# michaelnny/alpha_zero

Measured on AMD Instinct MI355X. Metric: self-play moves/sec (whole node), 9x9 Go @ 200 sims/move, higher is better.
Workload: dtype fp32-class evaluator (f16 hi+lo pairs, 3 MFMA products, fp32 accumulate) / f32-f64 tree

## Files before the change

alpha_zero_amd/csrc/azsp_hip.hip:

```cpp
#include <hip/hip_runtime.h>
#include <stdlib.h>

#include <type_traits>

#include "azsp_impl.h"
#include "az_conv64.h"
#include "az_conv19.h"
#include "az_conv_sp.h"
#include "az_conv_sp17.h"
#include "az_resblock_sp17.h"
#include "az_conv_sp2.h"
#include "az_conv_spg.h"
#include "az_stem_spg.h"

static hipError_t g_last = hipSuccess;
#define AZ_HIP(x) ((g_last = (x)) == hipSuccess ? 0 : -1)

template <int N, int GAME, class Op>
__global__ void __launch_bounds__(256) k_game(const AzCfg c, const AzMem m, const Op op, const int g0, const int g1) {
    __shared__ typename Engine<WaveDev, N, GAME>::SC sc[4];
    const int wave = (int)(threadIdx.x >> 6);
    const int g = g0 + (int)blockIdx.x * 4 + wave;
    if (g >= g1) return;
    Engine<WaveDev, N, GAME> e(c, m, g, sc[wave]);
    op(e);
}

__global__ void __launch_bounds__(256) k_dihedral(const DihedralArgs a, long long total) {
    for (long long t = (long long)blockIdx.x * blockDim.x + threadIdx.x; t < total; t += (long long)gridDim.x * blockDim.x)
        az_dihedral_elem(a, t);
}

__global__ void __launch_bounds__(256) k_replay_gather(const ReplayGatherArgs a, long long total) {
    for (long long t = (long long)blockIdx.x * blockDim.x + threadIdx.x; t < total; t += (long long)gridDim.x * blockDim.x)
        az_replay_gather_elem(a, t);
}

__global__ void __launch_bounds__(256) k_bias_act(const BiasActArgs a) {
    for (long long i = (long long)blockIdx.x * blockDim.x + threadIdx.x; i < a.nvec; i += (long long)gridDim.x * blockDim.x)
        az_bias_act_vec(a, i);
}

__global__ void __launch_bounds__(1024) k_harvest_scan(const int* __restrict__ len, int* __restrict__ ofs, int* __restrict__ counts, int n2, int rot,
                                                        int cap, int max_games) {
    __shared__ int ss[1024], sg[1024], best[2];
    const int t = (int)threadIdx.x, per = (n2 + 1023) / 1024, lo = t * per < n2 ? t * per : n2, hi = lo + per < n2 ? lo + per : n2;
    int s = 0, g = 0;
    for (int i = lo; i < hi; ++i) {
        const int l = len[(i + rot) % n2];
        s += l;
        g += l > 0;
    }
    ss[t] = s;
    sg[t] = g;
    if (t < 2) best[t] = 0;
    __syncthreads();
    for (int d = 1; d < 1024; d <<= 1) {
        const int a = t >= d ? ss[t - d] : 0, b = t >= d ? sg[t - d] : 0;
        __syncthreads();
        ss[t] += a;
        sg[t] += b;
        __syncthreads();
    }
    int mine[2] = {0, 0};
    az_harvest_scan_range(len, ofs, n2, rot, cap, max_games, lo, hi, ss[t] - s, sg[t] - g, mine);
    if (mine[1] > 0) {
        atomicMax(&best[0], mine[0]);
        atomicMax(&best[1], mine[1]);
    }
    __syncthreads();
    if (t < 2) counts[t] = best[t];
}

namespace azb {
void* alloc(size_t n) {
    void* p = nullptr;
    if (AZ_HIP(hipMalloc(&p, n))) return nullptr;
    if (AZ_HIP(hipMemset(p, 0, n))) {
        hipFree(p);
        return nullptr;
    }
    return p;
}
void release(void* p) { (void)hipFree(p); }
int h2d(void* d, const void* s, size_t n, void* st) {
    if (AZ_HIP(hipMemcpyAsync(d, s, n, hipMemcpyHostToDevice, (hipStream_t)st))) return -1;
    return AZ_HIP(hipStreamSynchronize((hipStream_t)st));
}
int d2h(void* d, const void* s, size_t n, void* st) {
    if (AZ_HIP(hipMemcpyAsync(d, s, n, hipMemcpyDeviceToHost, (hipStream_t)st))) return -1;
    return AZ_HIP(hipStreamSynchronize((hipStream_t)st));
}
int zero(void* d, size_t n, void* st) { return AZ_HIP(hipMemsetAsync(d, 0, n, (hipStream_t)st)); }
int sync(void* st) { return AZ_HIP(hipStreamSynchronize((hipStream_t)st)); }
void* host_alloc(size_t n) {
    void* p = nullptr;
    return AZ_HIP(hipHostMalloc(&p, n, hipHostMallocDefault)) ? nullptr : p;
}
void host_release(void* p) { (void)hipHostFree(p); }
int set_device(int dev) {
    int n = 0;
    if (AZ_HIP(hipGetDeviceCount(&n)) || n < 1) return -1;
    return AZ_HIP(hipSetDevice(dev));
}
const char* backend_error() { return hipGetErrorString(g_last); }
template <class K, class... A> static int launch_k(K* kernel, unsigned grid, unsigned block, size_t lds, void* st, const A&... args) {
    hipLaunchKernelGGL(kernel, dim3(grid), dim3(block), lds, (hipStream_t)st, args...);
    return AZ_HIP(hipGetLastError());
}
template <class F> static int with_flag(bool flag, F&& f) { return flag ? f(std::true_type{}) : f(std::false_type{}); }
template <class F> static int with_flag(bool f0, bool f1, F&& f) {
    return with_flag(f0, [&](auto F0) { return with_flag(f1, [&](auto F1) { return f(decltype(F0){}, F1); }); });
}
static int cu_count() {
    static int n_cu = 0;
    if (n_cu == 0) {
        int dev = 0;
        hipDeviceProp_t prop;
        if (hipGetDevice(&dev) != hipSuccess || hipGetDeviceProperties(&prop, dev) != hipSuccess) return -1;
        n_cu = prop.multiProcessorCount > 0 ? prop.multiProcessorCount : 256;
    }
    return n_cu;
}
static int persistent_grid(long long units, int k = 1) {
    const int n_cu = cu_count();
    if (n_cu < 0) return -1;
    const long long slots = n_cu / k > 0 ? n_cu / k : 1;
    return k * (int)(units < slots ? units : slots);
}
template <int N, int GAME, class Op> int launch(const AzCfg& c, const AzMem& m, const Op& op, void* st, int g0, int g1) {
    return launch_k(k_game<N, GAME, Op>, (unsigned)((g1 - g0 + 3) / 4), 256, 0, st, c, m, op, g0, g1);
}
int launch_dihedral(const DihedralArgs& a, long long total, void* st) {
    long long blocks = (total + 255) / 256;
    if (blocks > 2048) blocks = 2048;
    return launch_k(k_dihedral, (unsigned)blocks, 256, 0, st, a, total);
}
int launch_replay_gather(const ReplayGatherArgs& a, long long total, void* st) {
    long long blocks = (total + 255) / 256;
    if (blocks > 256 * 16) blocks = 256 * 16;
    return launch_k(k_replay_gather, (unsigned)blocks, 256, 0, st, a, total);
}
int launch_harvest_scan(const int* len, int* ofs, int* counts, int n2, int rot, int cap, int max_games, void* st) {
    return launch_k(k_harvest_scan, 1, 1024, 0, st, len, ofs, counts, n2, rot, cap, max_games);
}
int launch_bias_act(const BiasActArgs& a, void* st) {
    long long blocks = (a.nvec + 255) / 256;
    if (blocks > 256 * 32) blocks = 256 * 32;
    return launch_k(k_bias_act, (unsigned)blocks, 256, 0, st, a);
}
int launch_conv3x3_tiled(const void* x, const void* w, const float* bias, const void* res, void* y, long long boards, int S, int C,
                         int relu, void* st, int f16) {
    if (f16 && (S != CV_S || C != CV_C)) return 1;
    const auto xb = (const unsigned char*)x, rb = (const unsigned char*)res;
    const auto wb = (const unsigned short*)w;
    const auto yb = (unsigned char*)y;
    if (C == C6_C && (S == 17 || S == 9)) {
        const long long ntiles = S == 17 ? boards : (boards + 2) / 3;
        const int grid = persistent_grid(ntiles);
        if (grid < 0) return -1;
        return with_flag(S == 17, res != nullptr, [&](auto G17, auto RES) {
            return launch_k(k_conv3x3_t64<C6Geo<G17 ? 17 : 9>, RES, 8>, grid, CW_THREADS, 0, st, xb, wb, bias, rb, yb, (int)ntiles, relu);
        });
    }
    if (S == C9_S && C == 256) {
        static const bool two_launch = getenv("AZSP_CONV19_TWO_LAUNCH") != nullptr;
        const int grid = persistent_grid(boards, two_launch ? 4 : 8);
        if (grid < 0) return -1;
        if (x == y || res == y) return 1;
        if (!two_launch) {
            return with_flag(res != nullptr, [&](auto RES) {
                return launch_k(k_conv3x3_op19q<RES>, grid, CW_THREADS, 0, st, xb, wb, bias, rb, yb, (int)boards, relu);
            });
        }
        const int rc = with_flag(res != nullptr, [&](auto RES) {
            return launch_k(k_conv3x3_hb19<RES, 16>, grid, CW_THREADS, 0, st, xb, wb, bias, rb, yb, (int)boards, 0, 1, 256, 0, 32, 0);
        });
        if (rc) return rc;
        return launch_k(k_conv3x3_hb19<true, 16>, grid, CW_THREADS, 0, st, xb, wb, bias, (const unsigned char*)yb, yb, (int)boards, relu, 0, 256, 128, 32, 16);
    }
    if (S != CV_S || C != CV_C) return 1;
    const long long ntiles = (boards + CV_TB - 1) / CV_TB;
    const int grid = persistent_grid(ntiles);
    if (grid < 0) return -1;
    return with_flag(res != nullptr, f16 != 0, [&](auto RES, auto F16) {
        return launch_k(k_conv3x3_tiled<RES, 16, F16>, grid, CW_THREADS, 0, st, xb, wb, bias, rb, yb, (int)ntiles, relu);
    });
}
int launch_resblock_tiled(const void* x, const void* w1, const float* b1, const void* w2, const float* b2, void* y, long long boards, int S, int C,
                          void* st) {
    if (C != C6_C || (S != 17 && S != 9)) return 1;
    const long long ntiles = S == 17 ? boards : (boards + 2) / 3;
    const int grid = persistent_grid(ntiles);
    if (grid < 0) return -1;
    return with_flag(S == 17, [&](auto G17) {
        return launch_k(k_resblock64<C6Geo<G17 ? 17 : 9>>, grid, CW_THREADS, 0, st, (const unsigned char*)x, (const unsigned short*)w1, b1,
                        (const unsigned short*)w2, b2, (unsigned char*)y, (int)ntiles);
    });
}
int launch_stem_tiled(const void* x, const void* w, const float* bias, void* y, long long boards, int S, int C, int pad, int relu, void* st, int f16) {
    if (f16 && (S != CV_S || C != CV_C || pad != 1)) return 1;
    const bool t64 = C == C6_C && ((S == 13 && pad == 3) || (S == 9 && pad == 1)), go19 = S == C9_S && C == 256 && pad == 1;
    if (!t64 && !go19 && (S != CV_S || C != CV_C || pad != 1)) return 1;
    const long long ntiles = t64 ? (S == 13 ? boards : (boards + 2) / 3) : go19 ? boards : (boards + CV_TB - 1) / CV_TB;
    const int grid = persistent_grid(ntiles, go19 ? 4 : 1);
    if (grid < 0) return -1;
    const auto xb = (const unsigned char*)x, nores = (const unsigned char*)nullptr;
    const auto wb = (const unsigned short*)w;
    const auto yb = (unsigned char*)y;
    if (t64)
        return with_flag(S == 13, [&](auto G17) {
            return launch_k(k_conv3x3_t64<C6Geo<G17 ? 17 : 9>, false, 4>, grid, CW_THREADS, 0, st, xb, wb, bias, nores, yb, (int)ntiles, relu);
        });
    if (go19) return launch_k(k_conv3x3_hb19<false, 4>, grid, CW_THREADS, 0, st, xb, wb, bias, nores, yb, (int)boards, relu, 1, 32, 0, 4, 0);
    return with_flag(f16 != 0, [&](auto F16) {
        return launch_k(k_conv3x3_tiled<false, 4, F16>, grid, CW_THREADS, 0, st, xb, wb, bias, nores, yb, (int)ntiles, relu);
    });
}
int launch_head_tiled(const void* x, const float* w, const float* bias, void* pol, void* val, long long boards, int S, int C, int npol, int nval,
                      int pol_stride, int val_stride, void* st, int f16) {
    if (C % 8 || C > 1024 || npol + nval != 3) return 1;
    const long long npos = boards * S * S;
    return with_flag(f16 != 0, [&](auto F16) {
        return launch_k(k_head_tiled<3, F16>, (unsigned)((npos + 255) / 256), 256, 0, st, (const unsigned char*)x, w, bias, (unsigned short*)pol,
                        (unsigned short*)val, npos, npol, C, S * S, cv_tile_boards(S) * S * S, pol_stride, val_stride);
    });
}
template <int T1, int T2, bool F16> static int launch_fc_heads_t(const FcHeadsArgs& a, void* st) {
    return launch_k(k_fc_heads<T1, T2, F16>, (unsigned)((a.boards + 127) / 128), 256, 0, st, (const unsigned short*)a.pol, (const unsigned short*)a.val,
                    (const unsigned short*)a.wp, a.bp, a.ks1, (const unsigned short*)a.w1, a.b1, a.ks2, a.w2, a.b2, a.priors, a.values, a.boards, a.A);
}
int launch_fc_heads(const FcHeadsArgs& a, void* st) {
    const int nt1 = (a.A + 31) / 32, nt2 = (a.F + 31) / 32;
    if (a.f16) return nt1 == 3 && nt2 == 4 ? launch_fc_heads_t<3, 4, true>(a, st) : 1;
    if (nt1 == 3 && nt2 == 2) return launch_fc_heads_t<3, 2, false>(a, st);
    if (nt1 == 3 && nt2 == 4) return launch_fc_heads_t<3, 4, false>(a, st);
    if (nt1 == 6 && nt2 == 2) return launch_fc_heads_t<6, 2, false>(a, st);
    if (nt1 == 6 && nt2 == 4) return launch_fc_heads_t<6, 4, false>(a, st);
    if (nt1 == 12 && nt2 == 8) return launch_fc_heads_t<12, 8, false>(a, st);
    return 1;
}
int launch_tile_layout(const void* src, void* dst, long long boards, int S, int C, int to_tiled, void* st) {
    if (C % 8 || S < 1) return 1;
    const int nch = C / 8, tile_rows = cv_tile_boards(S) * S * S;
    const long long nchunks = boards * S * S * nch;
    return launch_k(k_tile_layout, (unsigned)((nchunks + 255) / 256), 256, 0, st, (const unsigned char*)src, (unsigned char*)dst, nchunks, to_tiled, nch,
                    tile_rows);
}
int launch_split_layout(const void* src, void* dst, long long boards, int S, int C, int to_split, void* st, unsigned* range) {
    if (C % 8 || S < 1) return 1;
    const long long nchunks = boards * S * S * (C / 8);
    return launch_k(k_split_layout, (unsigned)((nchunks + 255) / 256), 256, 0, st, (const unsigned char*)src, (unsigned char*)dst, nchunks, to_split, C / 8,
                    S * S, range);
}
template <bool RES, int NCH, int NCG, bool XLO0 = false>
static int launch_sp(const void* x, const void* w, const float* bias, const void* res, void* y, long long boards, int relu, void* st, unsigned* range) {
    const int grid = persistent_grid(boards, NCG);
    if (grid < 0) return -1;
    return launch_k(k_conv3x3_sp<RES, NCH, NCG, XLO0>, grid, CW_THREADS, 0, st, (const unsigned char*)x, (const _Float16*)w, bias, (const unsigned char*)res,
                    (unsigned char*)y, (int)boards, relu, range);
}
template <bool RES, int NCH, bool XLO0 = false>
static int launch_sp17(const void* x, const void* w, const float* bias, const void* res, void* y, long long boards, int relu, void* st, unsigned* range) {
    const int grid = persistent_grid(boards);
    if (grid < 0) return -1;
    return launch_k(k_conv3x3_sp17<RES, NCH, XLO0>, grid, CW_THREADS, 0, st, (const unsigned char*)x, (const _Float16*)w, bias, (const unsigned char*)res,
                    (unsigned char*)y, (int)boards, relu, range);
}
template <bool RES, int KSUB, int NT, int NJ, int HALVES>
static int launch_spg_t(const void* x, const void* w, const float* bias, const void* res, void* y, long long boards, int S, int C, int relu, void* st,
                        unsigned* range) {
    const long long nct = ((long long)S * S + 15) / 16, items = boards * ((nct + NJ - 1) / NJ) * (C / (16 * NT)), grid = (items + 3) / 4;
    if (grid > 0x7fffffffLL) return 1;
    return launch_k(k_conv3x3_spg<RES, KSUB, NT, NJ, HALVES>, (unsigned)grid, 256, 0, st, (const unsigned char*)x, (const _Float16*)w, bias,
                    (const unsigned char*)(RES ? res : nullptr), (unsigned char*)y, (int)boards, S, C, relu, range);
}
template <bool RES, int KSUB, int NT, int HALVES>
static int launch_spgw_t(const void* x, const void* w, const float* bias, const void* res, void* y, long long boards, int S, int C, int relu, void* st,
                         unsigned* range) {
    const long long nct = ((long long)S * S + 15) / 16, grid = (boards * ((nct + 2) / 3) * (C / (64 * NT)) + 7) / 8 * 8;
    if (grid > 0x7fffffffLL || C % (64 * NT)) return 1;
    return launch_k(k_conv3x3_spgw<RES, KSUB, NT, HALVES>, (unsigned)grid, 256, 0, st, (const unsigned char*)x, (const _Float16*)w, bias,
                    (const unsigned char*)(RES ? res : nullptr), (unsigned char*)y, (int)boards, S, C, relu, range);
}
template <int KSUB, int HALVES>
static int launch_spg_k(const void* x, const void* w, const float* bias, const void* res, void* y, long long boards, int S, int C, int relu, void* st,
                        unsigned* range, bool latency) {
    constexpr int NT = KSUB == 2 ? 1 : 2;
    return with_flag(res != nullptr, [&](auto RES) {
        return latency ? launch_spg_t<RES, KSUB, 1, 2, HALVES>(x, w, bias, res, y, boards, S, C, relu, st, range)
                       : launch_spgw_t<RES, KSUB, NT, HALVES>(x, w, bias, res, y, boards, S, C, relu, st, range);
    });
}
static int launch_spg(const void* x, const void* w, const float* bias, const void* res, void* y, long long boards, int S, int C, int relu, void* st,
                      unsigned* range, bool latency, int halves) {
    if (S < 3 || S > 64 || boards < 1 || boards > 0x7fffffffLL) return 1;
    if (C == 64) return launch_spg_k<2, 1>(x, w, bias, res, y, boards, S, C, relu, st, range, latency);
    if (C == 128)
        return halves == 2 ? launch_spg_k<4, 2>(x, w, bias, res, y, boards, S, C, relu, st, range, latency)
                           : launch_spg_k<4, 1>(x, w, bias, res, y, boards, S, C, relu, st, range, latency);
    if (C == 256) return launch_spg_k<8, 1>(x, w, bias, res, y, boards, S, C, relu, st, range, latency);
    return 1;
}
static constexpr long long SPG_DEFAULT_WAVES = 1024;
static long long& spg_max_waves() {
    static long long n = [] {
        const char* e = getenv("AZSP_SPG_MAX_WAVES");
        const long long v = e ? atoll(e) : SPG_DEFAULT_WAVES;
        return v < 0 ? 0LL : v;
    }();
    return n;
}
static bool small_batch(long long boards, int S, int C) { return boards * ((((long long)S * S + 15) / 16 + 1) / 2) * (C / 16) <= spg_max_waves(); }
long long small_batch_waves(long long n) {
    const long long old = spg_max_waves();
    if (n >= 0) spg_max_waves() = n;
    return old;
}
int launch_conv3x3_split(const void* x, const void* w, const float* bias, const void* res, void* y, long long boards, int S, int C, int relu,
                         void* st, unsigned* range) {
    const bool sp17 = S == Sp17Geo::S && C == 64, sp9 = S == SpGeo9::S && (C == 128 || C == 64), small = small_batch(boards, S, C);
    if (!(sp17 || sp9) || small) return launch_spg(x, w, bias, res, y, boards, S, C, relu, st, range, small, sp9 && C == 128 ? 2 : 1);
    if (sp17)
        return with_flag(res != nullptr, [&](auto RES) { return launch_sp17<RES, 8>(x, w, bias, res, y, boards, relu, st, range); });
    if (C == 64) return with_flag(res != nullptr, [&](auto RES) { return launch_sp<RES, 8, 1>(x, w, bias, res, y, boards, relu, st, range); });
    const int grid = persistent_grid(boards, 2);
    if (grid < 0) return -1;
    return with_flag(res != nullptr, [&](auto RES) {
        return launch_k(k_conv3x3_sp2<RES>, grid, CW_THREADS, 0, st, (const unsigned char*)x, (const _Float16*)w, bias, (const unsigned char*)res,
                        (unsigned char*)y, (int)boards, relu, range);
    });
}
enum Scratch {
    SCRATCH_SPG_BLOCK,
    SCRATCH_SP9_TAIL,
    SCRATCH_COUNT
};
static constexpr long long SPG_SCRATCH_BOARDS = 256;
static void* device_scratch(Scratch which, size_t bytes) {
    static void* buf[SCRATCH_COUNT][16] = {};
    int dev = 0;
    if (hipGetDevice(&dev) != hipSuccess || dev < 0 || dev >= 16) return nullptr;
    if (!buf[which][dev] && AZ_HIP(hipMalloc(&buf[which][dev], bytes))) return nullptr;
    return buf[which][dev];
}
int launch_resblock_split(const void* x, const void* w1, const float* b1, const void* w2, const float* b2, void* y, long long boards, int S, int C,
                          void* st, unsigned* range) {
    if (C != 64 || (S != Sb17::S && S != Sb9::S)) return 1;
    const long long pairs = boards / 2;
    const int grid = persistent_grid(S == Sb9::S ? pairs : boards);
    if (grid < 0) return -1;
    if (small_batch(boards, S, C) && boards <= SPG_SCRATCH_BOARDS) {
        void* mid = device_scratch(SCRATCH_SPG_BLOCK, (size_t)SPG_SCRATCH_BOARDS * 2 * 8 * Sb17::S * Sb17::S * 16);
        if (!mid) return -1;
        const int rc = launch_spg(x, w1, b1, nullptr, mid, boards, S, C, 1, st, range, true, 1);
        if (rc) return rc;
        return launch_spg(mid, w2, b2, x, y, boards, S, C, 1, st, range, true, 1);
    }
    const auto xb = (const unsigned char*)x;
    const auto yb = (unsigned char*)y;
    if (S == Sb17::S) return launch_k(k_resblock_sp<Sb17, 6>, grid, CW_THREADS, 0, st, xb, (const _Float16*)w1, b1, (const _Float16*)w2, b2, yb, (int)boards, range);
    if (pairs > 0 && launch_k(k_resblock_sp<Sb9, 6>, grid, CW_THREADS, 0, st, xb, (const _Float16*)w1, b1, (const _Float16*)w2, b2, yb, (int)pairs, range)) return -1;
    if (!(boards & 1)) return 0;
    void* mid = device_scratch(SCRATCH_SP9_TAIL, (size_t)Sb9::GTILEB);
    if (!mid) return -1;
    const size_t off = (size_t)(boards - 1) * Sb9::GTILEB;
    const int rc = launch_sp<false, 8, 1>(xb + off, w1, b1, nullptr, mid, 1, 1, st, range);
    if (rc) return rc;
    return launch_sp<true, 8, 1>(mid, w2, b2, xb + off, yb + off, 1, 1, st, range);
}
int launch_split_features(const float* src, void* dst, long long boards, int S, int cin, void* st, unsigned* range) {
    if (cin < 1 || cin > 32 || S < 1) return 1;
    const long long nitems = boards * 4 * S * S;
    return launch_k(k_split_features, (unsigned)((nitems + 255) / 256), 256, 0, st, src, (unsigned char*)dst, nitems, cin, S * S, range);
}
template <bool XLO0>
static int launch_stem_spg(const void* x, const void* w, const float* bias, void* y, long long boards, int n, int C, int pad, int relu, void* st,
                           unsigned* range) {
    constexpr int NT = 1, NJ = 2;
    const int off = pad - 1, S = n + 2 * off;
    if ((pad != 1 && pad != 3) || n < 1 || S < 3 || S > 64 || (C != 64 && C != 128 && C != 256) || boards < 1 || boards > 0x7fffffffLL) return 1;
    const long long nct = ((long long)S * S + 15) / 16, items = boards * ((nct + NJ - 1) / NJ) * (C / (16 * NT)), grid = (items + 3) / 4;
    if (grid > 0x7fffffffLL) return 1;
    return launch_k(k_stem_spg<XLO0, NT, NJ>, (unsigned)grid, 256, 0, st, (const unsigned char*)x, (const _Float16*)w, bias, (unsigned char*)y, (int)boards,
                    n, off, C, relu, range);
}
static constexpr bool STEM_SPG_DEFAULT_SMALL = false;
int launch_stem_split(const void* x, const void* w, const float* bias, void* y, long long boards, int S, int C, int pad, int relu, void* st,
                      int x_lo_zero, unsigned* range) {
    const bool sp17 = S == 13 && C == 64 && pad == 3;
    const bool sp9 = S == SpGeo9::S && (C == 128 || C == 64) && pad == 1;
    const bool small = (pad == 1 || pad == 3) && small_batch(boards, S + 2 * (pad - 1), C) && (STEM_SPG_DEFAULT_SMALL || spg_max_waves() > SPG_DEFAULT_WAVES);
    return with_flag(x_lo_zero != 0, [&](auto XLO0) {
        if (!(sp17 || sp9) || small) return launch_stem_spg<XLO0>(x, w, bias, y, boards, S, C, pad, relu, st, range);
        if (sp17) return launch_sp17<false, 4, XLO0>(x, w, bias, nullptr, y, boards, relu, st, range);
        return C == 128 ? launch_sp<false, 4, 2, XLO0>(x, w, bias, nullptr, y, boards, relu, st, range)
                        : launch_sp<false, 4, 1, XLO0>(x, w, bias, nullptr, y, boards, relu, st, range);
    });
}
int split_range_read(const unsigned* rec, unsigned out[2], int reset, void* st) {
    void* p = (void*)rec;
    if (!p && AZ_HIP(hipGetSymbolAddress(&p, HIP_SYMBOL(g_sp_range)))) return -1;
    if (AZ_HIP(hipMemcpyAsync(out, p, 2 * sizeof(unsigned), hipMemcpyDeviceToHost, (hipStream_t)st))) return -1;
    if (reset && AZ_HIP(hipMemsetAsync(p, 0, 2 * sizeof(unsigned), (hipStream_t)st))) return -1;
    return AZ_HIP(hipStreamSynchronize((hipStream_t)st));
}
template <int BPB> static int launch_head_split_bpb(const HeadSplitArgs& a, void* st) {
    const int P2 = a.S * a.S;
    const size_t lds = (size_t)(BPB * (3 * ((P2 + 3) & ~3) + a.A + a.F)) * sizeof(float);
    if (lds > 64 * 1024) return 1;
    return launch_k(k_head_split<BPB>, (unsigned)((a.boards + BPB - 1) / BPB), 256, lds, st, (const unsigned char*)a.x, a.hw, a.hb, a.wp_t, a.bp, a.w1_t, a.b1, a.w2,
                    a.b2, a.priors, a.values, a.boards, a.C, P2, a.A, a.F, a.npol);
}
int launch_head_split(const HeadSplitArgs& a, void* st) {
    if (a.C % 8 || a.npol < 1 || a.npol > 2) return 1;
    return launch_head_split_bpb<4>(a, st);
}
}
```

Baseline: 6672.

## Add persistent double-buffered stem kernel for 9x9 boards with 128 channels

Adds a dedicated stem convolution kernel for the 9x9, 128-channel case. It runs as a persistent grid sized to the CU count and walks over boards. The next board's input is prefetched into registers and written to a second LDS buffer while the current board is computed, so global load latency overlaps with MFMA work. Filter weights and bias stay in registers across boards instead of being reloaded per tile. The cost is higher register pressure and lower occupancy, plus a new hand-written code path for the default 9x9 configuration.

```diff
diff --git a/alpha_zero_amd/csrc/az_stem_sp9.h b/alpha_zero_amd/csrc/az_stem_sp9.h
--- /dev/null
+++ b/alpha_zero_amd/csrc/az_stem_sp9.h
@@ -0,0 +1,141 @@
+#pragma once
+#include "az_conv_sp.h"
+
+#if defined(__HIPCC__)
+template <bool XLO0> __global__ void __launch_bounds__(CW_THREADS, XLO0 ? 2 : 1)
+k_stem_sp9(const unsigned char* __restrict__ x, const _Float16* __restrict__ w, const float* __restrict__ bias, unsigned char* __restrict__ y, int nboards,
+           int relu, unsigned* range) {
+    typedef SpGeo9 G;
+    constexpr int C = 128, CIN = 32, NCH = 4, NPL = XLO0 ? 1 : 2;
+    constexpr int LBLK = G::CELLS * 16, LPLANE = NCH * LBLK, LBUF = NPL * LPLANE;
+    constexpr int GBLK = G::P2 * 16, XPLANE = NCH * GBLK, XTILE = 2 * XPLANE;
+    constexpr int YPLANE = (C / 8) * GBLK, YTILE = 2 * YPLANE;
+    constexpr int NCELL = NPL * NCH * G::P2, NLD = (NCELL + CW_THREADS - 1) / CW_THREADS;
+    constexpr int NT = 2, NJ = 2, NCT = G::NCT + 1;
+    static_assert(NCT % NJ == 0, "a board is NCT / NJ units of NJ column tiles");
+    static_assert(LBUF % 256 == 0, "both buffers start on the bank phase sp_map9 was generated for");
+    static_assert(LPLANE + 3 * LBLK + (G::CELLS + 1) * 16 <= 65536 && (G::P2 + 3 * G::P2) * 16 < 65536, "lane offsets fit 16 bits");
+    __shared__ __attribute__((aligned(1024))) unsigned char lds[2 * LBUF + 16];
+    const int tid = threadIdx.x, lane = tid & 63, l15 = lane & 15, kg = lane >> 4;
+    const int wave = __builtin_amdgcn_readfirstlane(tid >> 6);
+    for (int i = tid; i < (2 * LBUF + 16) / 16; i += CW_THREADS) *(cv_u32x4*)(lds + i * 16) = (cv_u32x4){0u, 0u, 0u, 0u};
+
+    unsigned soff[NLD], doff[NLD];
+    bool sok[NLD];
+#pragma unroll
+    for (int i = 0; i < NLD; ++i) {
+        const int c = tid + CW_THREADS * i;
+        sok[i] = c < NCELL;
+        const int cc = sok[i] ? c : 0, s = cc / G::P2, p = cc - s * G::P2;
+        soff[i] = (unsigned)(cc * 16);
+        doff[i] = (unsigned)(s * LBLK + (G::CELL0 + G::PITCH * (p / G::S) + p % G::S) * 16);
+    }
+    cv_u32x4 pre[NLD];
+    {
+        const unsigned char* src = x + (size_t)blockIdx.x * XTILE;
+#pragma unroll
+        for (int i = 0; i < NLD; ++i) pre[i] = *(const cv_u32x4*)(src + soff[i]);
+    }
+    sp_f16x8 wf[2][9][NT];
+#pragma unroll
+    for (int pl = 0; pl < 2; ++pl)
+#pragma unroll
+        for (int tap = 0; tap < 9; ++tap)
+#pragma unroll
+            for (int t = 0; t < NT; ++t)
+                wf[pl][tap][t] = *(const sp_f16x8*)(w + ((size_t)((pl * 9 + tap) * C + wave * 32 + 8 * (l15 >> 2) + 4 * t + (l15 & 3))) * CIN + kg * 8);
+    c6_f32x4 bv[NT];
+#pragma unroll
+    for (int t = 0; t < NT; ++t)
+#pragma unroll
+        for (int e = 0; e < 4; ++e) bv[t][e] = bias[wave * 32 + 8 * kg + 4 * t + e];
+    const float lo_clamp = relu ? 0.0f : -SP_F16_MAX;
+    unsigned lmap[NCT];
+#pragma unroll
+    for (int j = 0; j < NCT; ++j) {
+        const int pos = j < G::NCT ? sp_map9.pos[j * 16 + l15] : G::CORNER;
+        lmap[j] = (unsigned)((G::PITCH * (pos / G::S) + pos % G::S) * 16 + kg * LBLK) | ((unsigned)(pos * 16 + kg * GBLK) << 16);
+    }
+    const bool live5 = l15 == 0;
+    CV_BARRIER();
+#pragma unroll
+    for (int i = 0; i < NLD; ++i)
+        if (sok[i]) *(cv_u32x4*)(lds + doff[i]) = pre[i];
+    CV_BARRIER();
+
+    float mx = 0.0f;
+    auto unit = [&](auto UC, const unsigned char* Xs, unsigned char* yb) __attribute__((always_inline)) {
+        constexpr int u = decltype(UC)::value, j0 = u * NJ;
+        c6_f32x4 am[NT][NJ], ac[NT][NJ];
+#pragma unroll
+        for (int t = 0; t < NT; ++t)
+#pragma unroll
+            for (int j = 0; j < NJ; ++j) am[t][j] = bv[t], ac[t][j] = (c6_f32x4){0.0f, 0.0f, 0.0f, 0.0f};
+        cp_for_each([&](auto TC) __attribute__((always_inline)) {
+            constexpr int tap = decltype(TC)::value, off = ((tap / 3) * G::PITCH + tap % 3) * 16;
+            constexpr bool ctap = tap == 1 || tap == 2 || tap == 4 || tap == 5;
+            sp_f16x8 bh[NJ], bl[NJ];
+#pragma unroll
+            for (int j = 0; j < NJ; ++j)
+                if (j0 + j < G::NCT || ctap) {
+                    bh[j] = *(const sp_f16x8*)(Xs + (lmap[j0 + j] & 0xffffu) + off);
+                    if constexpr (!XLO0) bl[j] = *(const sp_f16x8*)(Xs + (lmap[j0 + j] & 0xffffu) + off + LPLANE);
+                }
+#pragma unroll
+            for (int j = 0; j < NJ; ++j)
+                if (j0 + j < G::NCT || ctap) {
+#pragma unroll
+                    for (int t = 0; t < NT; ++t) {
+                        am[t][j] = __builtin_amdgcn_mfma_f32_16x16x32_f16(wf[0][tap][t], bh[j], am[t][j], 0, 0, 0);
+                        if constexpr (!XLO0) ac[t][j] = __builtin_amdgcn_mfma_f32_16x16x32_f16(wf[0][tap][t], bl[j], ac[t][j], 0, 0, 0);
+                        ac[t][j] = __builtin_amdgcn_mfma_f32_16x16x32_f16(wf[1][tap][t], bh[j], ac[t][j], 0, 0, 0);
+                    }
+                }
+        }, typename CpMakeSeq<9>::type{});
+#pragma unroll
+        for (int j = 0; j < NJ; ++j) {
+            unsigned hp[2 * NT], lp[2 * NT];
+#pragma unroll
+            for (int t = 0; t < NT; ++t)
+#pragma unroll
+                for (int pr = 0; pr < 2; ++pr) {
+                    float e0 = fmaf(ac[t][j][2 * pr], SP_INV_SCALE, am[t][j][2 * pr]), e1 = fmaf(ac[t][j][2 * pr + 1], SP_INV_SCALE, am[t][j][2 * pr + 1]);
+                    const float m2 = sp_max3_abs(mx, e0, e1);
+                    mx = (j0 + j < G::NCT || live5) ? m2 : mx;
+                    e0 = __builtin_amdgcn_fmed3f(e0, lo_clamp, SP_F16_MAX);
+                    e1 = __builtin_amdgcn_fmed3f(e1, lo_clamp, SP_F16_MAX);
+                    const unsigned h = sp_cvt_pk(e0, e1);
+                    const float s0 = sp_mix_diff<0>(h, e0), s1 = sp_mix_diff<1>(h, e1);
+                    hp[2 * t + pr] = h;
+                    lp[2 * t + pr] = sp_scale_cvt_hi(sp_scale_cvt_lo(s0), s1);
+                }
+            if (j0 + j < G::NCT || live5) {
+                const unsigned o = lmap[j0 + j] >> 16;
+                *(cv_u32x4*)(yb + o) = (cv_u32x4){hp[0], hp[1], hp[2], hp[3]};
+                *(cv_u32x4*)(yb + YPLANE + o) = (cv_u32x4){lp[0], lp[1], lp[2], lp[3]};
+            }
+        }
+    };
+
+    const int nslot = (int)gridDim.x;
+    int it = 0;
+    for (int tile = (int)blockIdx.x; tile < nboards; tile += nslot, ++it) {
+        const int buf = it & 1;
+        const bool has_next = tile + nslot < nboards;
+        {
+            const unsigned char* src = x + (size_t)(has_next ? tile + nslot : tile) * XTILE;
+#pragma unroll
+            for (int i = 0; i < NLD; ++i) pre[i] = *(const cv_u32x4*)(src + soff[i]);
+        }
+        const unsigned char* Xs = lds + buf * LBUF;
+        unsigned char* yb = y + (size_t)tile * YTILE + (size_t)(wave * 4) * GBLK;
+        cp_for_each([&](auto UC) __attribute__((always_inline)) { unit(UC, Xs, yb); }, typename CpMakeSeq<NCT / NJ>::type{});
+        unsigned char* Xn = lds + (buf ^ 1) * LBUF;
+#pragma unroll
+        for (int i = 0; i < NLD; ++i)
+            if (sok[i]) *(cv_u32x4*)(Xn + doff[i]) = pre[i];
+        CV_BARRIER();
+    }
+    sp_range_report(mx, range);
+}
+#endif
diff --git a/alpha_zero_amd/csrc/azsp_hip.hip b/alpha_zero_amd/csrc/azsp_hip.hip
--- a/alpha_zero_amd/csrc/azsp_hip.hip
+++ b/alpha_zero_amd/csrc/azsp_hip.hip
@@ -12,6 +12,7 @@
 #include "az_conv_sp2.h"
 #include "az_conv_spg.h"
 #include "az_stem_spg.h"
+#include "az_stem_sp9.h"
 
 static hipError_t g_last = hipSuccess;
 #define AZ_HIP(x) ((g_last = (x)) == hipSuccess ? 0 : -1)
@@ -385,6 +386,14 @@
     return launch_k(k_stem_spg<XLO0, NT, NJ>, (unsigned)grid, 256, 0, st, (const unsigned char*)x, (const _Float16*)w, bias, (unsigned char*)y, (int)boards,
                     n, off, C, relu, range);
 }
+template <bool XLO0>
+static int launch_stem_sp9(const void* x, const void* w, const float* bias, void* y, long long boards, int relu, void* st, unsigned* range) {
+    const int n_cu = cu_count();
+    if (n_cu < 0) return -1;
+    const long long slots = (long long)n_cu * (XLO0 ? 2 : 1);
+    return launch_k(k_stem_sp9<XLO0>, (unsigned)(boards < slots ? boards : slots), CW_THREADS, 0, st, (const unsigned char*)x, (const _Float16*)w, bias,
+                    (unsigned char*)y, (int)boards, relu, range);
+}
 static constexpr bool STEM_SPG_DEFAULT_SMALL = false;
 int launch_stem_split(const void* x, const void* w, const float* bias, void* y, long long boards, int S, int C, int pad, int relu, void* st,
                       int x_lo_zero, unsigned* range) {
@@ -394,7 +403,7 @@
     return with_flag(x_lo_zero != 0, [&](auto XLO0) {
         if (!(sp17 || sp9) || small) return launch_stem_spg<XLO0>(x, w, bias, y, boards, S, C, pad, relu, st, range);
         if (sp17) return launch_sp17<false, 4, XLO0>(x, w, bias, nullptr, y, boards, relu, st, range);
-        return C == 128 ? launch_sp<false, 4, 2, XLO0>(x, w, bias, nullptr, y, boards, relu, st, range)
+        return C == 128 ? launch_stem_sp9<XLO0>(x, w, bias, y, boards, relu, st, range)
                         : launch_sp<false, 4, 1, XLO0>(x, w, bias, nullptr, y, boards, relu, st, range);
     });
 }
```

After: 6702 (median of 6 runs). No clear change (+0.4%).
